# ohsnyt/bzip2-rust

Hardware: AMD Instinct MI355X
Metric: compress MB/s at -9 (900 KB blocks), 1/2/4/8 MI355X; bit-exact vs C bzip2 (higher is better)
Workload: dtype u8; 1 GPU; 1024 MiB per GPU synthetic text at -9 (1194 blocks on this rank), BASELINE configs[2]; raw_bytes_total=1073741824, blocks_rank0=1194, compressed_bytes=323302688

## Files before the change

### bzip2-rust_amd/csrc/bzx_api.hip

```cpp
#include <string.h>
#include <chrono>
#include <new>
#include "bzx_host.h"
#include "bzx_wg.h"

extern "C" const char *bzx_version(void) { return "bzx 0.1 (gfx950)"; }

extern "C" const char *bzx_strerror(int code)
{
    switch (code) {
    case BZX_OK: return "ok";
    case BZX_E_NODEVICE: return "no HIP device";
    case BZX_E_PARAM: return "bad parameter";
    case BZX_E_NOMEM: return "out of memory";
    case BZX_E_OUTBUF: return "output buffer too small";
    case BZX_E_HIP: return "HIP runtime error";
    case BZX_E_STATE: return "bad call sequence";
    case BZX_E_DATA: return "damaged or invalid bzip2 data";
    default: return "unknown error";
    }
}

extern "C" const char *bzx_last_error(const bzx_ctx *ctx) { return ctx ? ctx->err.c_str() : ""; }

// ... 31 lines not shown
    if (nslab <= ctx->cap_slabs) return BZX_OK;
    ctx->slabs.clear();
    ctx->cap_slabs = 0;
    const uint32_t cap = nslab < 16 ? 16 : nslab;
    if ((rc = dev_alloc(ctx, ctx->slabs, &ctx->d_in, (size_t)cap * BZX_BLK_STRIDE))) return rc;
    if ((rc = dev_alloc(ctx, ctx->slabs, &B.bwt, (size_t)cap * BZX_BLK_STRIDE))) return rc;
    if ((rc = dev_alloc(ctx, ctx->slabs, &B.rank, (size_t)cap * BZX_BLK_STRIDE))) return rc;
    if ((rc = dev_alloc(ctx, ctx->slabs, &B.mtfv, (size_t)cap * BZX_BLK_STRIDE))) return rc;
    if ((rc = dev_alloc(ctx, ctx->slabs, &B.freq, (size_t)cap * 260))) return rc;
    if ((rc = dev_alloc(ctx, ctx->slabs, &B.in_use, (size_t)cap * 256))) return rc;
    if ((rc = dev_alloc(ctx, ctx->slabs, &B.len, (size_t)cap * 6 * 260))) return rc;
    if ((rc = dev_alloc(ctx, ctx->slabs, &B.code, (size_t)cap * 6 * 260))) return rc;
    if ((rc = dev_alloc(ctx, ctx->slabs, &B.selector, (size_t)cap * BZX_SEL_STRIDE))) return rc;
    if ((rc = dev_alloc(ctx, ctx->slabs, &B.selector_mtf, (size_t)cap * BZX_SEL_STRIDE))) return rc;
    if ((rc = dev_alloc(ctx, ctx->slabs, &B.gbits, (size_t)cap * BZX_SEL_STRIDE))) return rc;
    if ((rc = dev_alloc(ctx, ctx->slabs, &B.pk, (size_t)cap * BZX_PK_STRIDE))) return rc;
    if ((rc = dev_alloc(ctx, ctx->slabs, &B.rec_a, (size_t)cap * BZX_MAX_N))) return rc;
    if ((rc = dev_alloc(ctx, ctx->slabs, &B.rec_b, (size_t)cap * BZX_MAX_N))) return rc;
    if ((rc = dev_alloc(ctx, ctx->slabs, &B.bk_list, (size_t)cap * BZX_BK_PER_BLOCK))) return rc;
    B.bk_cap = cap * BZX_BK_PER_BLOCK;
    if ((rc = dev_alloc(ctx, ctx->slabs, &B.rk_list, (size_t)B.bk_cap * 2))) return rc;
    if ((rc = dev_alloc(ctx, ctx->slabs, &B.deep_list, (size_t)cap * BZX_DEEP_PER_BLOCK * 4 * 3))) return rc;
    if ((rc = dev_alloc(ctx, ctx->slabs, &B.isa2, (size_t)cap * 2 * BZX_MAX_N))) return rc;
    B.rk_blocks = cap;
    B.hpos = reinterpret_cast<uint32_t *>(B.rec_a);
    B.hpos_stride = 2 * BZX_MAX_N;
    if ((rc = dev_alloc(ctx, ctx->slabs, &ctx->d_outbuf, (size_t)cap * (BZX_OUT_STRIDE / 4)))) return rc;
    ctx->cap_slabs = cap;
    return BZX_OK;
}
// ... 204 lines not shown
        Br.redo = 2;
        Br.ctr_bwt = BZX_CTR_RESUME_FETCH;
        bzx_launch_bwt(Br, grid_for(ctx, nblk, per_cu), ctx->stream);
        bzx_launch_periodic(B, ctx->n_slots < 64 ? ctx->n_slots : 64, ctx->stream);
    }
    HIP_TRY(ctx, hipEventRecord(ctx->ev[1], ctx->stream));
    if ((stages & STG_MTF) && nblk) bzx_launch_mtf(B, grid_for(ctx, nblk, 1), ctx->stream);
    HIP_TRY(ctx, hipEventRecord(ctx->ev[2], ctx->stream));
    if ((stages & STG_HUF) && nblk) bzx_launch_huffman(B, grid_for(ctx, nblk, 3), ctx->stream);
    HIP_TRY(ctx, hipEventRecord(ctx->ev[3], ctx->stream));
    if (stages & STG_EMIT) {
        if (out_level < 0) {
            B.out = (uint32_t *)d_stream_out;
            bzx_launch_layout(B, 0, 0, ctx->d_scalars, ctx->stream, d_phase);
            HIP_TRY(ctx, hipMemsetAsync(d_stream_out, 0, stream_cap, ctx->stream));
            if (nblk) bzx_launch_emit(B, grid_for(ctx, nblk, 2), ctx->stream);
        } else if (out_level == 0) {
            B.out = ctx->d_outbuf;
            bzx_launch_layout(B, 0, (uint64_t)BZX_OUT_STRIDE * 8, ctx->d_scalars, ctx->stream);
            HIP_TRY(ctx, hipMemsetAsync(ctx->d_outbuf, 0, (size_t)nblk * BZX_OUT_STRIDE, ctx->stream));
            if (nblk) bzx_launch_emit(B, grid_for(ctx, nblk, 2), ctx->stream);
        } else {
            B.out = (uint32_t *)d_stream_out;
            bzx_launch_layout(B, 32, 0, ctx->d_scalars, ctx->stream);
            HIP_TRY(ctx, hipMemcpyAsync(ctx->h_scalars, ctx->d_scalars, sizeof(uint64_t), hipMemcpyDeviceToHost,
                                        ctx->stream));
            HIP_TRY(ctx, hipStreamSynchronize(ctx->stream));
            const uint64_t out_bytes = (ctx->h_scalars[0] + 80 + 7) >> 3;
            const uint64_t need = (out_bytes + 3) & ~3ull;
            ctx->h_scalars[1] = out_bytes;
            if (need > stream_cap) {
                ctx->err = "output buffer too small for the compressed stream";
                return BZX_E_OUTBUF;
            }
            HIP_TRY(ctx, hipMemsetAsync(d_stream_out, 0, need, ctx->stream));
            if (nblk) bzx_launch_emit(B, grid_for(ctx, nblk, 2), ctx->stream);
            bzx_launch_stream_frame(B, out_level, ctx->d_scalars, ctx->d_scalars + 1, ctx->stream);
        }
    }
    HIP_TRY(ctx, hipEventRecord(ctx->ev[4], ctx->stream));
    HIP_TRY(ctx, hipMemcpyAsync(ctx->h_counters, ctx->d_counters, 64 * sizeof(uint32_t), hipMemcpyDeviceToHost, ctx->stream));
    HIP_TRY(ctx, hipGetLastError());
    return BZX_OK;
}

int bzx_ctx_split_scratch(bzx_ctx *ctx, size_t bytes, void **p)
{
    if (!ctx->split_ws.reserve(bytes)) {
        ctx->err = "hipMalloc(split scratch) failed";
        return BZX_E_NOMEM;
    }
// ... 639 lines not shown
    HIP_TRY(ctx, hipStreamSynchronize(ctx->stream));
    ctx->shard_packed_max = world <= 64 ? ctx->h_scalars[3] * 4 : 0;
    const uint64_t out_bytes = (ctx->h_scalars[0] + 80 + 7) >> 3;
    const uint64_t need = ctx->h_scalars[2] * 4;
    if (need > cap) {
        ctx->err = "packed buffer too small for this rank's blocks";
        return BZX_E_OUTBUF;
    }
    HIP_TRY(ctx, hipMemsetAsync(d_packed, 0, need, ctx->stream));
    HIP_TRY(ctx, hipMemsetAsync(ctx->d_counters, 0, 64 * sizeof(uint32_t), ctx->stream));
    B.out = (uint32_t *)d_packed;
    B.nblk = mine;
    B.blk_first = rank;
    B.blk_step = world;
    B.packed = 1;
    if (mine) bzx_launch_emit(B, grid_for(ctx, mine, 2), ctx->stream);
    B.packed = 0;
    HIP_TRY(ctx, hipEventRecord(ctx->ev[4], ctx->stream));
    HIP_TRY(ctx, hipEventRecord(ctx->ev[7], ctx->stream));
    if (nblk) HIP_TRY(ctx, hipMemcpyAsync(ctx->h_blk, B.blk, nblk * sizeof(BzxBlock), hipMemcpyDeviceToHost, ctx->stream));
    HIP_TRY(ctx, hipStreamSynchronize(ctx->stream));
    HIP_TRY(ctx, hipGetLastError());
    B.nblk = nblk;
    B.blk_first = 0;
    B.blk_step = 1;
    *packed_len = (size_t)need;
    *stream_len = (size_t)out_bytes;
    bzx_stats &st = ctx->stats;
    collect_stage_times(ctx);
    st.nblk = mine;
    ctx->stats_batch = false;
// ... 134 lines not shown
```

### bzip2-rust_amd/csrc/bzx_batch.hip

```cpp
#include <hip/hip_runtime.h>
#include <string.h>
#include <new>
#include "bzx_host.h"
#include "bzx_rle1.h"

#define BT_NT 1024
#define BX_NT 256
#define BX_WORDS 5
static_assert(sizeof(bzx_index_entry) == BX_WORDS * 8 && (BX_NT * BX_WORDS) % 2 == 0, "index entries: whole 16-byte vectors per workgroup");

__device__ __forceinline__ uint64_t bt_carry(const BzxBatchWs &ws, const BzxSeg &s, uint64_t tile)
{
    const uint64_t v = ws.tile_rs[tile], base = s.tile0 * RL_TILE;
    return v > base ? v - base : 0;
}

__global__ __launch_bounds__(RL_NT) void bzx_bt_runstart_kernel(BzxBatchWs ws)
{
    __shared__ uint64_t scratch[RL_NT / 64];
    for (uint64_t tile = blockIdx.x; tile < ws.ntiles; tile += gridDim.x) {
        const BzxSeg s = ws.seg[ws.tile_seg[tile]];
        bool any4;
        const uint64_t tot = bzx_tile_runstart(s.raw, s.len, tile - s.tile0, scratch, any4);
        if (threadIdx.x == 0) {
// ... 508 lines not shown
        }
        if (end > cap4) {
            ctx->err = "output buffer too small for the batch (input " + std::to_string(i0) + " onwards does not fit; "
                       "bzx_compress_batch_bound always fits)";
            return BZX_E_OUTBUF;
        }
        fold_blocks(stt, ctx->h_blk, 0, nb, 1);
        for (uint32_t i = i0; i < i1; i++) {
            stt.raw_bytes += lens[i];
            stt.out_bits += (uint64_t)out_lens[i] * 8;
        }
        stt.nblk += nb;
        HIP_TRY(ctx, hipEventRecord(ctx->ev_bt[1], st));
        HIP_TRY(ctx, hipMemsetAsync((uint8_t *)d_out + base, 0, end - base, st));
        B.nblk = nb;
        if (nb) bzx_launch_emit(B, grid_for(ctx, nb, 2), st);
        bzx_batch_launch_frame(ws, i0, i1, rb0, B.blk, d_out, level, st);
        HIP_TRY(ctx, hipEventRecord(ctx->ev_bt[2], st));
        HIP_TRY(ctx, hipGetLastError());
        emit_pending = true;
        base = end;
        i0 = i1;
    }
    HIP_TRY(ctx, hipEventRecord(ctx->ev[7], st));
    HIP_TRY(ctx, hipStreamSynchronize(st));
    if (emit_pending) {
        float ms = 0.f;
        (void)hipEventElapsedTime(&ms, ctx->ev_bt[1], ctx->ev_bt[2]);
        stt.ms_emit += ms;
    }
    (void)hipEventElapsedTime(&stt.ms_total, ctx->ev[5], ctx->ev[7]);
// ... 131 lines not shown
```

### bzip2-rust_amd/csrc/bzx_device.h

```cpp
#pragma once
#include <stdint.h>
#include <stddef.h>

#define BZX_MAX_N 900000u
#define BZX_BLK_STRIDE 900096u
#define BZX_MAX_ALPHA 258
#define BZX_G_SIZE 50
#define BZX_N_ITERS 4
#define BZX_MAX_SEL 18002
#define BZX_SEL_STRIDE 18048

#define BZX_IN_RAW (1ull << 63)
#define BZX_ST_PERIODIC 1u
#define BZX_ST_REDO 2u
#define BZX_ST_RESUME 4u
#define BZX_ST_DC_RANDOMISED 0x400u
#define DC_ERR_HEADER 0x100u
#define DC_ERR_DATA 0x200u
#define DC_SKIP 0x800u
#define DC_MAGIC_BLOCK 0x314159265359ull
#define DC_MAGIC_EOS 0x177245385090ull
#ifndef RK_ROUNDS
#define RK_ROUNDS 11
#endif
#define RK_COARSE 0x80000000u
// ... 71 lines not shown
    uint32_t *plist;
    const uint8_t *in;
    const uint8_t *raw;
    uint8_t *bwt;
    uint8_t *rank;
    uint32_t *hpos;
    uint32_t hpos_stride;
    uint16_t *mtfv;
    uint32_t *freq;
    uint8_t *in_use;
    uint8_t *len;
    uint32_t *code;
    uint8_t *selector;
    uint8_t *selector_mtf;
    uint16_t *gbits;
    uint32_t *out;
    BzxSortWs *sort_ws;
    uint8_t *pk;
    uint64_t *rec_a;
    uint64_t *rec_b;
    BzxBucket *bk_list;
    uint32_t bk_cap;
    uint32_t bk_affine;
    uint32_t *redo_list;
    uint32_t *resume_list;
    uint32_t *rk_list;
    uint32_t *deep_list;
    uint32_t deep_cap;
    uint32_t deep_lvl;
    uint32_t *isa2;
// ... 73 lines not shown
```

### bzip2-rust_amd/csrc/bzx_emit.hip

```cpp
#include <hip/hip_runtime.h>
#include "bzx_host.h"
#include "bzx_wg.h"

#define EMIT_NT 512
#define EMIT_NW (EMIT_NT / 64)

struct BitW {
    uint32_t *out;
    uint64_t wi;
    uint64_t acc;
    uint32_t nacc;
    bool first;
    __device__ __forceinline__ void init(uint32_t *o, uint64_t bitpos)
    {
        out = o;
        wi = bitpos >> 5;
        nacc = (uint32_t)(bitpos & 31u);
        acc = 0;
        first = true;
    }
    __device__ __forceinline__ void flush_word(uint32_t w)
    {
        const uint32_t be = __builtin_bswap32(w);
        if (first) {
            if (be) atomicOr(&out[wi], be);
            first = false;
        } else {
            out[wi] = be;
        }
        wi++;
    }
    __device__ __forceinline__ void put(uint32_t nbits, uint32_t val)
    {
        if (nbits == 0) return;
        acc = (acc << nbits) | (uint64_t)val;
        nacc += nbits;
        if (nacc >= 32) {
            nacc -= 32;
            flush_word((uint32_t)(acc >> nacc));
            acc &= (1ull << nacc) - 1ull;
        }
    }
    __device__ __forceinline__ void finish()
    {
        if (nacc > 0) {
            const uint32_t be = __builtin_bswap32((uint32_t)(acc << (32 - nacc)));
            if (be) atomicOr(&out[wi], be);
        }
    }
};

__shared__ uint8_t e_len[6][BZX_MAX_ALPHA + 2];
__shared__ uint32_t e_code[6][BZX_MAX_ALPHA + 2];
__shared__ uint32_t e_cl[6][BZX_MAX_ALPHA + 2];
__shared__ __attribute__((aligned(16))) uint32_t e_tile[EMIT_NT * (BZX_G_SIZE / 2)];
__shared__ uint32_t e_tabbits[8];
__shared__ uint32_t e_scratch[2 * EMIT_NW];
__shared__ uint32_t e_bcast[4];

#define EMIT_STAMP(slot)                                                      \
    do {                                                                      \
        if (B.dbg && tid == 0) {                                              \
            const unsigned long long now_ = wall_clock64();                   \
            atomicAdd(&B.dbg[slot], now_ - t_last);                           \
            t_last = now_;                                                    \
        }                                                                     \
    } while (0)

__global__ __launch_bounds__(EMIT_NT) void bzx_emit_kernel(BzxBatch B)
{
    const uint32_t tid = threadIdx.x, lane = bzx_lane(), wave = bzx_wave();
    unsigned long long t_last = 0;

    for (;;) {
        if (tid == 0) e_bcast[0] = atomicAdd(&B.counters[3], 1u);
        __syncthreads();
        const uint32_t j_ = e_bcast[0];
        __syncthreads();
        if (j_ >= B.nblk) break;
        const uint32_t b = B.blk_first + j_ * B.blk_step;

        if (B.dbg && tid == 0) t_last = wall_clock64();
        const BzxBlock d = B.blk[b];
        const uint32_t alpha = d.n_in_use + 2, n_mtf = d.n_mtf, n_sel = d.n_selectors, n_groups = d.n_groups;
        const uint16_t *__restrict__ V = B.mtfv + BZX_SLAB(B, b) * BZX_BLK_STRIDE;
        const uint8_t *__restrict__ SEL = B.selector + BZX_SLAB(B, b) * BZX_SEL_STRIDE;
        const uint8_t *__restrict__ SELM = B.selector_mtf + BZX_SLAB(B, b) * BZX_SEL_STRIDE;
        const uint16_t *__restrict__ GB = B.gbits + BZX_SLAB(B, b) * BZX_SEL_STRIDE;
        uint32_t *out = B.out;

        const uint64_t ob = B.packed ? d.pack_word * 32 + (d.out_bit & 31u) : d.out_bit;
        const uint64_t o_map = ob + 105;
        const uint64_t o_ng = o_map + d.sec_bits[3];
        const uint64_t o_sel = o_ng + 18;
        const uint64_t o_tab = o_sel + d.sec_bits[0];
        const uint64_t o_pay = o_tab + d.sec_bits[1];

        for (uint32_t i = tid; i < 6 * 260; i += EMIT_NT) {
            const uint32_t t = i / 260, v = i % 260;
            if (v < BZX_MAX_ALPHA + 2) {
                e_len[t][v] = B.len[BZX_SLAB(B, b) * 6 * 260 + i];
                e_code[t][v] = B.code[BZX_SLAB(B, b) * 6 * 260 + i];
                e_cl[t][v] = B.code[BZX_SLAB(B, b) * 6 * 260 + i] | ((uint32_t)B.len[BZX_SLAB(B, b) * 6 * 260 + i] << 24);
            }
        }
        __syncthreads();

        if (tid == 0) {
            BitW w;
            w.init(out, ob);
            w.put(24, 0x314159u);
            w.put(24, 0x265359u);
            w.put(32, d.crc);
            w.put(1, 0);
            w.put(24, d.orig_ptr);
            uint32_t l1 = 0, words[16];
            for (uint32_t i = 0; i < 16; i++) {
                uint32_t wv = 0;
                for (uint32_t j = 0; j < 16; j++)
                    if (B.in_use[BZX_SLAB(B, b) * 256 + i * 16 + j]) wv |= 0x8000u >> j;
                words[i] = wv;
                if (wv) l1 |= 0x8000u >> i;
            }
            w.put(16, l1);
            for (uint32_t i = 0; i < 16; i++)
                if (words[i]) w.put(16, words[i]);
            w.put(3, n_groups);
            w.put(15, n_sel);
            w.finish();
        }

        EMIT_STAMP(48);
        {
            const uint32_t per = (n_sel + EMIT_NT - 1) / EMIT_NT;
            const uint32_t lo = tid * per < n_sel ? tid * per : n_sel;
            const uint32_t hi = lo + per < n_sel ? lo + per : n_sel;
            uint32_t my_bits = 0;
            for (uint32_t i = lo; i < hi; i++) my_bits += SELM[i] + 1u;
            uint32_t tot;
            const uint32_t ex = bzx_block_excl_sum<EMIT_NT>(my_bits, e_scratch, tot);
            if (hi > lo) {
                BitW w;
                w.init(out, o_sel + ex);
                for (uint32_t i = lo; i < hi; i++) {
                    const uint32_t j = SELM[i];
                    w.put(j + 1, ((1u << j) - 1u) << 1);
                }
                w.finish();
            }
        }

        EMIT_STAMP(49);
        if (lane == 0 && wave < n_groups) {
            uint32_t bits = 5;
            int32_t curr = e_len[wave][0];
            for (uint32_t i = 0; i < alpha; i++) {
                const int32_t l = e_len[wave][i];
                bits += 2u * (uint32_t)(l > curr ? l - curr : curr - l) + 1u;
                curr = l;
            }
            e_tabbits[wave] = bits;
        }
        __syncthreads();
        if (lane == 0 && wave < n_groups) {
            uint64_t pos = o_tab;
            for (uint32_t t = 0; t < wave; t++) pos += e_tabbits[t];
            BitW w;
            w.init(out, pos);
            int32_t curr = e_len[wave][0];
            w.put(5, (uint32_t)curr);
            for (uint32_t i = 0; i < alpha; i++) {
                const int32_t l = e_len[wave][i];
                while (curr < l) {
                    w.put(2, 2);
                    curr++;
                }
                while (curr > l) {
                    w.put(2, 3);
                    curr--;
                }
                w.put(1, 0);
            }
            w.finish();
        }

        __syncthreads();
        EMIT_STAMP(50);
        {
            if (tid == 0) e_bcast[1] = 0;
            __syncthreads();
            for (uint32_t g0 = 0; g0 < n_sel; g0 += EMIT_NT) {
                const uint32_t g = g0 + tid;
                const uint32_t carry = e_bcast[1];
                const uint32_t gb = g < n_sel ? (uint32_t)GB[g] : 0u;
                uint32_t tot;
                const uint32_t ex = bzx_block_excl_sum<EMIT_NT>(gb, e_scratch, tot);
                {
                    const uint4 *__restrict__ src = reinterpret_cast<const uint4 *>(V + (size_t)g0 * BZX_G_SIZE);
                    uint4 *dst = reinterpret_cast<uint4 *>(e_tile);
                    const uint32_t ng = n_sel - g0 < EMIT_NT ? n_sel - g0 : EMIT_NT;
                    const uint32_t nq = (ng * (BZX_G_SIZE / 2) + 3u) / 4u;
                    for (uint32_t i = tid; i < nq; i += EMIT_NT) dst[i] = src[i];
                }
                __syncthreads();
                if (g < n_sel) {
                    const uint32_t gs = g * BZX_G_SIZE;
                    const uint32_t cnt = (n_mtf - gs < BZX_G_SIZE) ? n_mtf - gs : BZX_G_SIZE;
                    const uint32_t *vp = e_tile + tid * (BZX_G_SIZE / 2);
                    const uint32_t *__restrict__ cl = e_cl[SEL[g]];
                    uint32_t vw[BZX_G_SIZE / 2];
#pragma unroll
                    for (uint32_t k = 0; k < BZX_G_SIZE / 2; k++) vw[k] = 2 * k < cnt ? vp[k] : 0u;
                    BitW w;
                    w.init(out, o_pay + carry + ex);
#pragma unroll
                    for (uint32_t k = 0; k < BZX_G_SIZE / 2; k++) {
                        const uint32_t c0 = 2 * k < cnt ? cl[vw[k] & 0xffffu] : 0u;
                        const uint32_t c1 = 2 * k + 1 < cnt ? cl[vw[k] >> 16] : 0u;
                        w.put(c0 >> 24, c0 & 0xffffffu);
                        w.put(c1 >> 24, c1 & 0xffffffu);
                    }
                    w.finish();
                }
                if (tid == 0) e_bcast[1] = carry + tot;
                __syncthreads();
            }
        }
        __syncthreads();
        EMIT_STAMP(51);
    }
}

__global__ __launch_bounds__(EMIT_NT) void bzx_layout_kernel(BzxBatch B, uint64_t first_bit, uint64_t stride_bits,
                                                            uint64_t *total, uint64_t *phase)
{
    __shared__ uint64_t l_wsum[EMIT_NW];
    __shared__ uint64_t l_carry;
    const uint32_t tid = threadIdx.x, lane = bzx_lane(), wave = bzx_wave();
    if (phase) first_bit = phase[0];
    if (tid == 0) l_carry = first_bit;
    __syncthreads();
    for (uint32_t b0 = 0; b0 < B.nblk; b0 += EMIT_NT) {
        const uint32_t b = b0 + tid;
        const uint64_t v = b < B.nblk ? B.blk[b].bits : 0ull;
        uint64_t x = v;
// ... 169 lines not shown
void bzx_launch_unpack(const BzxBatch &B, const uint32_t *packed, uint32_t first, uint32_t step, uint32_t nown,
                       uint32_t grid, hipStream_t stream)
{
    hipLaunchKernelGGL(bzx_unpack_kernel, dim3(grid), dim3(256), 0, stream, B, packed, first, step, nown);
}

void bzx_launch_bits_export(const BzxBatch &B, long long *bits, hipStream_t stream)
{
    hipLaunchKernelGGL(bzx_bits_export_kernel, dim3(64), dim3(256), 0, stream, B, bits);
}
void bzx_launch_bits_import(const BzxBatch &B, const long long *bits, hipStream_t stream)
{
    hipLaunchKernelGGL(bzx_bits_import_kernel, dim3(64), dim3(256), 0, stream, B, bits);
}

void bzx_launch_emit(const BzxBatch &B, uint32_t grid, hipStream_t stream)
{
    hipLaunchKernelGGL(bzx_emit_kernel, dim3(grid), dim3(EMIT_NT), 0, stream, B);
}

void bzx_launch_layout(const BzxBatch &B, uint64_t first_bit, uint64_t stride_bits, uint64_t *d_total_bits,
                       hipStream_t stream, uint64_t *d_phase)
{
    hipLaunchKernelGGL(bzx_layout_kernel, dim3(1), dim3(EMIT_NT), 0, stream, B, first_bit, stride_bits, d_total_bits,
                       d_phase);
}

void bzx_launch_stream_frame(const BzxBatch &B, int level, const uint64_t *d_total_bits, uint64_t *d_out_bytes,
                             hipStream_t stream)
{
    hipLaunchKernelGGL(bzx_stream_frame_kernel, dim3(1), dim3(256), 0, stream, B, level, d_total_bits, d_out_bytes);
}
// ... 1 lines not shown
```

### bzip2-rust_amd/csrc/bzx_host.h

```cpp
#pragma once
#include <hip/hip_runtime.h>
#include <condition_variable>
#include <mutex>
#include <string>
#include <vector>
#include "../../include/bzx.h"
#include "bzx_dc.h"
#include "bzx_device.h"
#include "bzx_mem.h"

struct BlockReq {
    const uint8_t *blk;
    size_t n;
    uint32_t crc;
    uint8_t *out;
    size_t cap;
    size_t out_len = 0;
    uint8_t pad = 0;
    int rc = 0;
    bool done = false;
};

struct bzx_ctx {
    int device = 0;
// ... 163 lines not shown
__host__ __device__ static inline uint32_t crc_fold(uint32_t comb, uint32_t crc) { return ((comb << 1) | (comb >> 31)) ^ crc; }

void bzx_launch_shift_bits(const uint32_t *d_in, uint32_t n_words, uint32_t p, uint32_t *d_out, uint32_t n_cu,
                           hipStream_t stream);

void bzx_launch_bwt(const BzxBatch &B, uint32_t grid, hipStream_t stream);
uint32_t bzx_bwt_max_blocks_per_cu();
void bzx_launch_bsplit(const BzxBatch &B, uint32_t grid, uint32_t grid_deep, hipStream_t stream);
void bzx_launch_bsort(const BzxBatch &B, uint32_t grid, hipStream_t stream);
void bzx_launch_brank(const BzxBatch &B, uint32_t grid, hipStream_t stream);
void bzx_launch_bgiant(const BzxBatch &B, uint32_t grid, hipStream_t stream);
uint32_t bzx_bsort_blocks_per_cu();
void bzx_launch_periodic(const BzxBatch &B, uint32_t grid, hipStream_t stream);
void bzx_launch_mtf(const BzxBatch &B, uint32_t grid, hipStream_t stream);
void bzx_launch_huffman(const BzxBatch &B, uint32_t grid, hipStream_t stream);
void bzx_launch_emit(const BzxBatch &B, uint32_t grid, hipStream_t stream);
void bzx_launch_layout(const BzxBatch &B, uint64_t first_bit, uint64_t stride_bits, uint64_t *d_total_bits,
                       hipStream_t stream, uint64_t *d_phase = nullptr);
void bzx_launch_stream_frame(const BzxBatch &B, int level, const uint64_t *d_total_bits, uint64_t *d_out_bytes,
                             hipStream_t stream);
void bzx_launch_bits_export(const BzxBatch &B, long long *bits, hipStream_t stream);
void bzx_launch_bits_import(const BzxBatch &B, const long long *bits, hipStream_t stream);
void bzx_launch_pack_layout(const BzxBatch &B, uint32_t first, uint32_t step, uint32_t nown, uint64_t *d_total,
                            hipStream_t stream);
void bzx_launch_pack_max(const BzxBatch &B, uint32_t world, uint64_t *d_out, hipStream_t stream);
void bzx_launch_zero_edges(const BzxBatch &B, const uint64_t *d_total, hipStream_t stream);
void bzx_launch_unpack(const BzxBatch &B, const uint32_t *packed, uint32_t first, uint32_t step, uint32_t nown,
                       uint32_t grid, hipStream_t stream);

int bzx_split_launch_boundaries(bzx_ctx *ctx, const uint8_t *d_raw, size_t len, int level, uint32_t max_blocks,
                                BzxSplitWs *ws_out);
// ... 18 lines not shown
```

### bzip2-rust_amd/csrc/bzx_huff.hip

```cpp
#include <hip/hip_runtime.h>
#include "bzx_host.h"
#include "bzx_wg.h"

#define HUF_NT 512
#define HUF_NW (HUF_NT / 64)

__shared__ uint32_t h_freq[BZX_MAX_ALPHA + 2];
__shared__ uint8_t h_len[6][BZX_MAX_ALPHA + 2];
__shared__ uint2 h_lenAB[BZX_MAX_ALPHA + 2];
__shared__ uint32_t h_rfreq[6][BZX_MAX_ALPHA + 2];
#define HUF_PK 9
#define HUF_PK_COPIES 8
#define HUF_PK_STRIDE 19
__shared__ unsigned long long h_pk[HUF_PK_COPIES * HUF_PK_STRIDE];
__shared__ __attribute__((aligned(16))) uint64_t h_heap[6][BZX_MAX_ALPHA + 2];
__shared__ int32_t h_weight[6][BZX_MAX_ALPHA + 2];
__shared__ int32_t h_parent[6][BZX_MAX_ALPHA * 2];
__shared__ uint32_t h_code[6][BZX_MAX_ALPHA + 2];
__shared__ uint32_t h_part[6][2];
__shared__ uint32_t h_scratch[2 * HUF_NW];
__shared__ uint32_t h_bcast[4];
__shared__ uint32_t h_acc[4];

__device__ void make_code_lengths(int t, int32_t alpha, int32_t max_len)
{
    uint64_t *heap = h_heap[t];
    int32_t *weight = h_weight[t], *parent = h_parent[t];
    const int32_t lane = (int32_t)bzx_lane();
    for (int32_t i = lane; i < alpha; i += 64) {
        const uint32_t f = h_rfreq[t][i];
        weight[i + 1] = (int32_t)((f == 0 ? 1u : f) << 8);
    }
    for (;;) {
        bzx_wave_sync();
        if (lane == 0) {
            int32_t n_nodes = alpha, n_heap = 0;
            heap[0] = 0;
// ... 86 lines not shown
#ifdef BZX_HIP_EMU
#define HUF_FORGET(x) do {} while (0)
#else
#define HUF_FORGET(x) asm volatile("" : "+v"(x))
#endif

#define HUF_STAMP(slot)                                                       \
    do {                                                                      \
        if (B.dbg && tid == 0) {                                              \
            const unsigned long long now_ = wall_clock64();                   \
            atomicAdd(&B.dbg[slot], now_ - t_last);                           \
            t_last = now_;                                                    \
        }                                                                     \
    } while (0)

#ifndef HUF_WAVES_PER_SIMD
#define HUF_WAVES_PER_SIMD 6
#endif
__global__ __launch_bounds__(HUF_NT) __attribute__((amdgpu_waves_per_eu(HUF_WAVES_PER_SIMD, HUF_WAVES_PER_SIMD))) void bzx_huff_kernel(BzxBatch B)
{
    const uint32_t tid = threadIdx.x, lane = bzx_lane(), wave = bzx_wave();
    unsigned long long t_last = 0;

    for (;;) {
        if (tid == 0) h_bcast[0] = atomicAdd(&B.counters[2], 1u);
        __syncthreads();
        const uint32_t j_ = bzx_uni(h_bcast[0]);
        __syncthreads();
        if (j_ >= B.nblk) break;
        const uint32_t b = B.blk_first + j_ * B.blk_step;

        if (B.dbg && tid == 0) t_last = wall_clock64();
        const uint32_t n_mtf = bzx_uni(B.blk[b].n_mtf);
        const uint32_t alpha = bzx_uni(B.blk[b].n_in_use) + 2;
        const uint16_t *__restrict__ V = B.mtfv + BZX_SLAB(B, b) * BZX_BLK_STRIDE;
        uint8_t *__restrict__ SEL = B.selector + BZX_SLAB(B, b) * BZX_SEL_STRIDE;
        uint8_t *__restrict__ SELM = B.selector_mtf + BZX_SLAB(B, b) * BZX_SEL_STRIDE;
        uint16_t *__restrict__ GB = B.gbits + BZX_SLAB(B, b) * BZX_SEL_STRIDE;
        const uint32_t n_sel = (n_mtf + BZX_G_SIZE - 1) / BZX_G_SIZE;
        const uint32_t n_groups = n_mtf < 200 ? 2u : n_mtf < 600 ? 3u : n_mtf < 1200 ? 4u : n_mtf < 2400 ? 5u : 6u;

        for (uint32_t i = tid; i < BZX_MAX_ALPHA + 2; i += HUF_NT) h_freq[i] = i < alpha ? B.freq[BZX_SLAB(B, b) * 260 + i] : 0u;
        if (tid < 4) h_acc[tid] = 0;
        __syncthreads();

        if (tid == 0) {
            int32_t n_part = (int32_t)n_groups, rem_f = (int32_t)n_mtf, gs = 0;
            while (n_part > 0) {
                const int32_t t_freq = rem_f / n_part;
                int32_t ge = gs - 1, a_freq = 0;
                while (a_freq < t_freq && ge < (int32_t)alpha - 1) {
                    ge++;
                    a_freq += (int32_t)h_freq[ge];
// ... 139 lines not shown
                for (int k = 0; k < BZX_G_SIZE; k++) {
                    const uint32_t sm = (sy[k >> 1] >> (16 * (k & 1))) & 0xffffu;
                    const uint2 l2 = h_lenAB[sm];
                    accA += l2.x;
                    accB += l2.y;
                }
                const uint32_t pick = bt < 3 ? accA : accB;
                const uint32_t acc = (pick >> (10 * (bt % 3))) & 1023u;
                GB[g] = (uint16_t)acc;
                my_bits += acc;
            }
            uint32_t tot;
            (void)bzx_block_excl_sum<HUF_NT>(my_bits, h_scratch, tot);
            if (tid == 0) h_acc[2] = tot;
        }

        HUF_STAMP(44);
        {
            const uint32_t per = (n_sel + HUF_NT - 1) / HUF_NT;
            const uint32_t lo = tid * per;
            const uint32_t hi = lo + per < n_sel ? lo + per : n_sel;
            uint32_t lp[6] = {0, 0, 0, 0, 0, 0};
            for (uint32_t i = lo; i < hi; i++) {
                const uint32_t sg = SEL[i];
#pragma unroll
                for (uint32_t t = 0; t < 6; t++)
                    if (sg == t) lp[t] = i + 1;
            }
#pragma unroll
            for (uint32_t t = 0; t < 6; t++) {
// ... 71 lines not shown
```

### include/bzx.h

```cpp
#ifndef BZX_H
#define BZX_H

#include <stddef.h>
#include <stdint.h>

#ifdef __cplusplus
extern "C" {
#endif

#define BZX_OK 0
#define BZX_E_NODEVICE (-1)
#define BZX_E_PARAM (-2)
#define BZX_E_NOMEM (-3)
#define BZX_E_OUTBUF (-4)
#define BZX_E_HIP (-5)
#define BZX_E_STATE (-6)
#define BZX_E_DATA (-7)

#define BZX_MAX_BLOCK 900000u

typedef struct bzx_ctx bzx_ctx;

const char *bzx_version(void);
const char *bzx_strerror(int code);
// ... 8 lines not shown
int bzx_compress_blocks(bzx_ctx *ctx, uint32_t nblk, const uint8_t *const *blks, const size_t *ns,
                        const uint32_t *crcs, uint8_t *const *outs, const size_t *caps, size_t *out_lens,
                        uint8_t *pads);

int bzx_stage_bwt(bzx_ctx *ctx, const uint8_t *blk, size_t n, uint8_t *bwt_out, uint32_t *orig_ptr,
                  uint32_t *status);
int bzx_stage_mtf(bzx_ctx *ctx, const uint8_t *bwt, size_t n, uint16_t *mtfv_out, uint32_t *n_mtf,
                  uint32_t freq_out[258], uint8_t in_use_out[256]);
int bzx_stage_huffman(bzx_ctx *ctx, const uint16_t *mtfv, uint32_t n_mtf, const uint32_t freq[258],
                      uint32_t alpha_size, uint32_t *n_groups, uint32_t *n_selectors, uint8_t *selectors,
                      uint8_t len_out[6][258], uint32_t code_out[6][258]);
struct bzx_block_info;
int bzx_stage_encode(bzx_ctx *ctx, const uint16_t *mtfv, uint32_t n_mtf, const uint32_t freq[258],
                     const uint8_t in_use[256], uint32_t orig_ptr, uint32_t crc, uint8_t *out, size_t cap,
                     size_t *out_len, uint8_t *pad_bits, uint8_t *selector_mtf, struct bzx_block_info *info);

int bzx_split_rle1(bzx_ctx *ctx, const uint8_t *raw, size_t len, int level, uint8_t *blocks_out,
                   uint32_t nblk_cap, uint32_t *ns, uint32_t *crcs, uint32_t *nblk);

int bzx_compress_device(bzx_ctx *ctx, const void *d_raw, size_t len, int level, void *d_out, size_t cap,
                        size_t *out_len);
int bzx_compress_buffer(bzx_ctx *ctx, const uint8_t *raw, size_t len, int level, uint8_t *out, size_t cap,
                        size_t *out_len);

size_t bzx_compress_batch_bound(uint32_t count, const size_t *lens);
int bzx_compress_batch_device(bzx_ctx *ctx, uint32_t count, const void *const *d_raws, const size_t *lens, int level,
                              void *d_out, size_t cap, size_t *out_offs, size_t *out_lens);
int bzx_compress_batch_buffer(bzx_ctx *ctx, uint32_t count, const uint8_t *const *raws, const size_t *lens, int level,
                              uint8_t *out, size_t cap, size_t *out_offs, size_t *out_lens);

// ... 203 lines not shown
```

Before: 30240 MB/s.

## Split emit into per-tile work items with LDS-staged bit packing

The Huffman kernel now computes per-tile prefix bit offsets for each block. With those offsets, the emit kernel can split a block into several independent work items of four 512-group tiles each, instead of one workgroup serially walking all tiles. Each tile is packed into an LDS staging buffer without global atomics, then written out as byteswapped vector stores, with atomics only at the boundary words. The next tile's inputs are prefetched into registers, and the grid is capped at two workgroups per CU. In exchange, there is extra LDS use and the code tables are reloaded once per work item.

```diff
diff --git a/bzip2-rust_amd/csrc/bzx_api.hip b/bzip2-rust_amd/csrc/bzx_api.hip
--- a/bzip2-rust_amd/csrc/bzx_api.hip
+++ b/bzip2-rust_amd/csrc/bzx_api.hip
@@ -69,6 +69,7 @@
     if ((rc = dev_alloc(ctx, ctx->slabs, &B.selector, (size_t)cap * BZX_SEL_STRIDE))) return rc;
     if ((rc = dev_alloc(ctx, ctx->slabs, &B.selector_mtf, (size_t)cap * BZX_SEL_STRIDE))) return rc;
     if ((rc = dev_alloc(ctx, ctx->slabs, &B.gbits, (size_t)cap * BZX_SEL_STRIDE))) return rc;
+    if ((rc = dev_alloc(ctx, ctx->slabs, &B.tbits, (size_t)cap * BZX_TILE_STRIDE))) return rc;
     if ((rc = dev_alloc(ctx, ctx->slabs, &B.pk, (size_t)cap * BZX_PK_STRIDE))) return rc;
     if ((rc = dev_alloc(ctx, ctx->slabs, &B.rec_a, (size_t)cap * BZX_MAX_N))) return rc;
     if ((rc = dev_alloc(ctx, ctx->slabs, &B.rec_b, (size_t)cap * BZX_MAX_N))) return rc;
@@ -303,12 +304,12 @@
             B.out = (uint32_t *)d_stream_out;
             bzx_launch_layout(B, 0, 0, ctx->d_scalars, ctx->stream, d_phase);
             HIP_TRY(ctx, hipMemsetAsync(d_stream_out, 0, stream_cap, ctx->stream));
-            if (nblk) bzx_launch_emit(B, grid_for(ctx, nblk, 2), ctx->stream);
+            if (nblk) bzx_launch_emit(B, (uint32_t)ctx->n_cu, ctx->stream);
         } else if (out_level == 0) {
             B.out = ctx->d_outbuf;
             bzx_launch_layout(B, 0, (uint64_t)BZX_OUT_STRIDE * 8, ctx->d_scalars, ctx->stream);
             HIP_TRY(ctx, hipMemsetAsync(ctx->d_outbuf, 0, (size_t)nblk * BZX_OUT_STRIDE, ctx->stream));
-            if (nblk) bzx_launch_emit(B, grid_for(ctx, nblk, 2), ctx->stream);
+            if (nblk) bzx_launch_emit(B, (uint32_t)ctx->n_cu, ctx->stream);
         } else {
             B.out = (uint32_t *)d_stream_out;
             bzx_launch_layout(B, 32, 0, ctx->d_scalars, ctx->stream);
@@ -323,7 +324,7 @@
                 return BZX_E_OUTBUF;
             }
             HIP_TRY(ctx, hipMemsetAsync(d_stream_out, 0, need, ctx->stream));
-            if (nblk) bzx_launch_emit(B, grid_for(ctx, nblk, 2), ctx->stream);
+            if (nblk) bzx_launch_emit(B, (uint32_t)ctx->n_cu, ctx->stream);
             bzx_launch_stream_frame(B, out_level, ctx->d_scalars, ctx->d_scalars + 1, ctx->stream);
         }
     }
@@ -993,7 +994,7 @@
     B.blk_first = rank;
     B.blk_step = world;
     B.packed = 1;
-    if (mine) bzx_launch_emit(B, grid_for(ctx, mine, 2), ctx->stream);
+    if (mine) bzx_launch_emit(B, (uint32_t)ctx->n_cu, ctx->stream);
     B.packed = 0;
     HIP_TRY(ctx, hipEventRecord(ctx->ev[4], ctx->stream));
     HIP_TRY(ctx, hipEventRecord(ctx->ev[7], ctx->stream));
diff --git a/bzip2-rust_amd/csrc/bzx_batch.hip b/bzip2-rust_amd/csrc/bzx_batch.hip
--- a/bzip2-rust_amd/csrc/bzx_batch.hip
+++ b/bzip2-rust_amd/csrc/bzx_batch.hip
@@ -546,7 +546,7 @@
         HIP_TRY(ctx, hipEventRecord(ctx->ev_bt[1], st));
         HIP_TRY(ctx, hipMemsetAsync((uint8_t *)d_out + base, 0, end - base, st));
         B.nblk = nb;
-        if (nb) bzx_launch_emit(B, grid_for(ctx, nb, 2), st);
+        if (nb) bzx_launch_emit(B, (uint32_t)ctx->n_cu, st);
         bzx_batch_launch_frame(ws, i0, i1, rb0, B.blk, d_out, level, st);
         HIP_TRY(ctx, hipEventRecord(ctx->ev_bt[2], st));
         HIP_TRY(ctx, hipGetLastError());
diff --git a/bzip2-rust_amd/csrc/bzx_device.h b/bzip2-rust_amd/csrc/bzx_device.h
--- a/bzip2-rust_amd/csrc/bzx_device.h
+++ b/bzip2-rust_amd/csrc/bzx_device.h
@@ -9,6 +9,10 @@
 #define BZX_N_ITERS 4
 #define BZX_MAX_SEL 18002
 #define BZX_SEL_STRIDE 18048
+#define BZX_EMIT_TILE 512u
+#define BZX_MAX_TILES ((BZX_MAX_SEL + BZX_EMIT_TILE - 1) / BZX_EMIT_TILE)
+#define BZX_TILE_STRIDE 40
+static_assert(BZX_MAX_TILES <= BZX_TILE_STRIDE, "a block's tile prefixes fit its stride of BzxBatch.tbits");
 
 #define BZX_IN_RAW (1ull << 63)
 #define BZX_ST_PERIODIC 1u
@@ -110,6 +114,7 @@
     uint8_t *selector;
     uint8_t *selector_mtf;
     uint16_t *gbits;
+    uint32_t *tbits;
     uint32_t *out;
     BzxSortWs *sort_ws;
     uint8_t *pk;
diff --git a/bzip2-rust_amd/csrc/bzx_emit.hip b/bzip2-rust_amd/csrc/bzx_emit.hip
--- a/bzip2-rust_amd/csrc/bzx_emit.hip
+++ b/bzip2-rust_amd/csrc/bzx_emit.hip
@@ -5,7 +5,15 @@
 #define EMIT_NT 512
 #define EMIT_NW (EMIT_NT / 64)
 
-struct BitW {
+#ifndef EMIT_TPI
+#define EMIT_TPI 4
+#endif
+#define EMIT_SLOTS ((BZX_MAX_TILES + EMIT_TPI - 1) / EMIT_TPI)
+static_assert(EMIT_NT == BZX_EMIT_TILE, "one lane per group of a tile");
+#define EMIT_STAGE_BITS (EMIT_NT * BZX_G_SIZE * 17u)
+#define EMIT_STAGE_WORDS ((EMIT_STAGE_BITS / 32u + 2u + 3u + 3u) & ~3u)
+
+template <bool GLOBAL> struct BitWT {
     uint32_t *out;
     uint64_t wi;
     uint64_t acc;
@@ -21,7 +29,7 @@
     }
     __device__ __forceinline__ void flush_word(uint32_t w)
     {
-        const uint32_t be = __builtin_bswap32(w);
+        const uint32_t be = GLOBAL ? __builtin_bswap32(w) : w;
         if (first) {
             if (be) atomicOr(&out[wi], be);
             first = false;
@@ -44,16 +52,17 @@
     __device__ __forceinline__ void finish()
     {
         if (nacc > 0) {
-            const uint32_t be = __builtin_bswap32((uint32_t)(acc << (32 - nacc)));
+            const uint32_t w = (uint32_t)(acc << (32 - nacc));
+            const uint32_t be = GLOBAL ? __builtin_bswap32(w) : w;
             if (be) atomicOr(&out[wi], be);
         }
     }
 };
+typedef BitWT<true> BitW;
 
 __shared__ uint8_t e_len[6][BZX_MAX_ALPHA + 2];
-__shared__ uint32_t e_code[6][BZX_MAX_ALPHA + 2];
 __shared__ uint32_t e_cl[6][BZX_MAX_ALPHA + 2];
-__shared__ __attribute__((aligned(16))) uint32_t e_tile[EMIT_NT * (BZX_G_SIZE / 2)];
+__shared__ __attribute__((aligned(16))) uint32_t e_stage[EMIT_STAGE_WORDS];
 __shared__ uint32_t e_tabbits[8];
 __shared__ uint32_t e_scratch[2 * EMIT_NW];
 __shared__ uint32_t e_bcast[4];
@@ -67,18 +76,51 @@
         }                                                                     \
     } while (0)
 
+__device__ __forceinline__ void emit_load_tile(const uint16_t *__restrict__ V, const uint16_t *__restrict__ GB,
+                                               const uint8_t *__restrict__ SEL, const uint32_t *__restrict__ TB, uint32_t t,
+                                               uint32_t n_sel, uint32_t (&vw)[BZX_G_SIZE / 2], uint32_t &gb, uint32_t &sel,
+                                               uint32_t &tb)
+{
+    const uint32_t g = t * EMIT_NT + threadIdx.x;
+    tb = TB[t];
+    gb = 0;
+    sel = 0;
+#pragma unroll
+    for (uint32_t k = 0; k < BZX_G_SIZE / 2; k++) vw[k] = 0;
+    if (g < n_sel) {
+        const uint32_t *__restrict__ vp = reinterpret_cast<const uint32_t *>(V + (size_t)g * BZX_G_SIZE);
+#pragma unroll
+        for (uint32_t k = 0; k < BZX_G_SIZE / 2; k++) vw[k] = vp[k];
+        gb = GB[g];
+        sel = SEL[g];
+    }
+}
+
 __global__ __launch_bounds__(EMIT_NT) void bzx_emit_kernel(BzxBatch B)
 {
     const uint32_t tid = threadIdx.x, lane = bzx_lane(), wave = bzx_wave();
     unsigned long long t_last = 0;
+    const uint32_t n_items = B.nblk * EMIT_SLOTS;
+    uint4 *stage4 = reinterpret_cast<uint4 *>(e_stage);
+    for (uint32_t i = tid; i < EMIT_STAGE_WORDS / 4; i += EMIT_NT) stage4[i] = make_uint4(0u, 0u, 0u, 0u);
 
     for (;;) {
-        if (tid == 0) e_bcast[0] = atomicAdd(&B.counters[3], 1u);
-        __syncthreads();
-        const uint32_t j_ = e_bcast[0];
-        __syncthreads();
-        if (j_ >= B.nblk) break;
-        const uint32_t b = B.blk_first + j_ * B.blk_step;
+        if (tid == 0) {
+            uint32_t id;
+            for (;;) {
+                id = atomicAdd(&B.counters[3], 1u);
+                if (id >= n_items || id % EMIT_SLOTS == 0) break;
+                const uint32_t bb = B.blk_first + (id / EMIT_SLOTS) * B.blk_step;
+                if ((id % EMIT_SLOTS) * (EMIT_TPI * EMIT_NT) < B.blk[bb].n_selectors) break;
+            }
+            e_bcast[0] = id;
+        }
+        __syncthreads();
+        const uint32_t id = bzx_uni(e_bcast[0]);
+        __syncthreads();
+        if (id >= n_items) break;
+        const uint32_t slot = id % EMIT_SLOTS;
+        const uint32_t b = B.blk_first + (id / EMIT_SLOTS) * B.blk_step;
 
         if (B.dbg && tid == 0) t_last = wall_clock64();
         const BzxBlock d = B.blk[b];
@@ -87,6 +129,7 @@
         const uint8_t *__restrict__ SEL = B.selector + BZX_SLAB(B, b) * BZX_SEL_STRIDE;
         const uint8_t *__restrict__ SELM = B.selector_mtf + BZX_SLAB(B, b) * BZX_SEL_STRIDE;
         const uint16_t *__restrict__ GB = B.gbits + BZX_SLAB(B, b) * BZX_SEL_STRIDE;
+        const uint32_t *__restrict__ TB = B.tbits + BZX_SLAB(B, b) * BZX_TILE_STRIDE;
         uint32_t *out = B.out;
 
         const uint64_t ob = B.packed ? d.pack_word * 32 + (d.out_bit & 31u) : d.out_bit;
@@ -96,139 +139,164 @@
         const uint64_t o_tab = o_sel + d.sec_bits[0];
         const uint64_t o_pay = o_tab + d.sec_bits[1];
 
+        const uint32_t n_tiles = (n_sel + EMIT_NT - 1) / EMIT_NT;
+        const uint32_t t0 = slot * EMIT_TPI, t1 = t0 + EMIT_TPI < n_tiles ? t0 + EMIT_TPI : n_tiles;
         for (uint32_t i = tid; i < 6 * 260; i += EMIT_NT) {
             const uint32_t t = i / 260, v = i % 260;
             if (v < BZX_MAX_ALPHA + 2) {
-                e_len[t][v] = B.len[BZX_SLAB(B, b) * 6 * 260 + i];
-                e_code[t][v] = B.code[BZX_SLAB(B, b) * 6 * 260 + i];
-                e_cl[t][v] = B.code[BZX_SLAB(B, b) * 6 * 260 + i] | ((uint32_t)B.len[BZX_SLAB(B, b) * 6 * 260 + i] << 24);
-            }
-        }
-        __syncthreads();
-
-        if (tid == 0) {
-            BitW w;
-            w.init(out, ob);
-            w.put(24, 0x314159u);
-            w.put(24, 0x265359u);
-            w.put(32, d.crc);
-            w.put(1, 0);
-            w.put(24, d.orig_ptr);
-            uint32_t l1 = 0, words[16];
-            for (uint32_t i = 0; i < 16; i++) {
-                uint32_t wv = 0;
-                for (uint32_t j = 0; j < 16; j++)
-                    if (B.in_use[BZX_SLAB(B, b) * 256 + i * 16 + j]) wv |= 0x8000u >> j;
-                words[i] = wv;
-                if (wv) l1 |= 0x8000u >> i;
-            }
-            w.put(16, l1);
-            for (uint32_t i = 0; i < 16; i++)
-                if (words[i]) w.put(16, words[i]);
-            w.put(3, n_groups);
-            w.put(15, n_sel);
-            w.finish();
-        }
-
-        EMIT_STAMP(48);
-        {
-            const uint32_t per = (n_sel + EMIT_NT - 1) / EMIT_NT;
-            const uint32_t lo = tid * per < n_sel ? tid * per : n_sel;
-            const uint32_t hi = lo + per < n_sel ? lo + per : n_sel;
-            uint32_t my_bits = 0;
-            for (uint32_t i = lo; i < hi; i++) my_bits += SELM[i] + 1u;
-            uint32_t tot;
-            const uint32_t ex = bzx_block_excl_sum<EMIT_NT>(my_bits, e_scratch, tot);
-            if (hi > lo) {
+                const uint8_t l = B.len[BZX_SLAB(B, b) * 6 * 260 + i];
+                if (slot == 0) e_len[t][v] = l;
+                e_cl[t][v] = B.code[BZX_SLAB(B, b) * 6 * 260 + i] | ((uint32_t)l << 24);
+            }
+        }
+        uint32_t vn[BZX_G_SIZE / 2], gbn, seln, tbn;
+        emit_load_tile(V, GB, SEL, TB, t0, n_sel, vn, gbn, seln, tbn);
+        bzx_lds_barrier();
+
+        if (slot == 0) {
+            if (tid == 0) {
                 BitW w;
-                w.init(out, o_sel + ex);
-                for (uint32_t i = lo; i < hi; i++) {
-                    const uint32_t j = SELM[i];
-                    w.put(j + 1, ((1u << j) - 1u) << 1);
+                w.init(out, ob);
+                w.put(24, 0x314159u);
+                w.put(24, 0x265359u);
+                w.put(32, d.crc);
+                w.put(1, 0);
+                w.put(24, d.orig_ptr);
+                uint32_t l1 = 0, words[16];
+                for (uint32_t i = 0; i < 16; i++) {
+                    uint32_t wv = 0;
+                    for (uint32_t j = 0; j < 16; j++)
+                        if (B.in_use[BZX_SLAB(B, b) * 256 + i * 16 + j]) wv |= 0x8000u >> j;
+                    words[i] = wv;
+                    if (wv) l1 |= 0x8000u >> i;
                 }
+                w.put(16, l1);
+                for (uint32_t i = 0; i < 16; i++)
+                    if (words[i]) w.put(16, words[i]);
+                w.put(3, n_groups);
+                w.put(15, n_sel);
                 w.finish();
             }
-        }
-
-        EMIT_STAMP(49);
-        if (lane == 0 && wave < n_groups) {
-            uint32_t bits = 5;
-            int32_t curr = e_len[wave][0];
-            for (uint32_t i = 0; i < alpha; i++) {
-                const int32_t l = e_len[wave][i];
-                bits += 2u * (uint32_t)(l > curr ? l - curr : curr - l) + 1u;
-                curr = l;
-            }
-            e_tabbits[wave] = bits;
-        }
-        __syncthreads();
-        if (lane == 0 && wave < n_groups) {
-            uint64_t pos = o_tab;
-            for (uint32_t t = 0; t < wave; t++) pos += e_tabbits[t];
-            BitW w;
-            w.init(out, pos);
-            int32_t curr = e_len[wave][0];
-            w.put(5, (uint32_t)curr);
-            for (uint32_t i = 0; i < alpha; i++) {
-                const int32_t l = e_len[wave][i];
-                while (curr < l) {
-                    w.put(2, 2);
-                    curr++;
-                }
-                while (curr > l) {
-                    w.put(2, 3);
-                    curr--;
-                }
-                w.put(1, 0);
-            }
-            w.finish();
-        }
-
-        __syncthreads();
-        EMIT_STAMP(50);
-        {
-            if (tid == 0) e_bcast[1] = 0;
-            __syncthreads();
-            for (uint32_t g0 = 0; g0 < n_sel; g0 += EMIT_NT) {
-                const uint32_t g = g0 + tid;
-                const uint32_t carry = e_bcast[1];
-                const uint32_t gb = g < n_sel ? (uint32_t)GB[g] : 0u;
+
+            EMIT_STAMP(48);
+            {
+                const uint32_t per = (n_sel + EMIT_NT - 1) / EMIT_NT;
+                const uint32_t lo = tid * per < n_sel ? tid * per : n_sel;
+                const uint32_t hi = lo + per < n_sel ? lo + per : n_sel;
+                uint32_t my_bits = 0;
+                for (uint32_t i = lo; i < hi; i++) my_bits += SELM[i] + 1u;
                 uint32_t tot;
-                const uint32_t ex = bzx_block_excl_sum<EMIT_NT>(gb, e_scratch, tot);
-                {
-                    const uint4 *__restrict__ src = reinterpret_cast<const uint4 *>(V + (size_t)g0 * BZX_G_SIZE);
-                    uint4 *dst = reinterpret_cast<uint4 *>(e_tile);
-                    const uint32_t ng = n_sel - g0 < EMIT_NT ? n_sel - g0 : EMIT_NT;
-                    const uint32_t nq = (ng * (BZX_G_SIZE / 2) + 3u) / 4u;
-                    for (uint32_t i = tid; i < nq; i += EMIT_NT) dst[i] = src[i];
-                }
-                __syncthreads();
-                if (g < n_sel) {
-                    const uint32_t gs = g * BZX_G_SIZE;
-                    const uint32_t cnt = (n_mtf - gs < BZX_G_SIZE) ? n_mtf - gs : BZX_G_SIZE;
-                    const uint32_t *vp = e_tile + tid * (BZX_G_SIZE / 2);
-                    const uint32_t *__restrict__ cl = e_cl[SEL[g]];
-                    uint32_t vw[BZX_G_SIZE / 2];
-#pragma unroll
-                    for (uint32_t k = 0; k < BZX_G_SIZE / 2; k++) vw[k] = 2 * k < cnt ? vp[k] : 0u;
+                const uint32_t ex = bzx_block_excl_sum_lds<EMIT_NT>(my_bits, e_scratch, tot);
+                if (hi > lo) {
                     BitW w;
-                    w.init(out, o_pay + carry + ex);
-#pragma unroll
-                    for (uint32_t k = 0; k < BZX_G_SIZE / 2; k++) {
-                        const uint32_t c0 = 2 * k < cnt ? cl[vw[k] & 0xffffu] : 0u;
-                        const uint32_t c1 = 2 * k + 1 < cnt ? cl[vw[k] >> 16] : 0u;
-                        w.put(c0 >> 24, c0 & 0xffffffu);
-                        w.put(c1 >> 24, c1 & 0xffffffu);
+                    w.init(out, o_sel + ex);
+                    for (uint32_t i = lo; i < hi; i++) {
+                        const uint32_t j = SELM[i];
+                        w.put(j + 1, ((1u << j) - 1u) << 1);
                     }
                     w.finish();
                 }
-                if (tid == 0) e_bcast[1] = carry + tot;
-                __syncthreads();
-            }
-        }
-        __syncthreads();
+            }
+
+            EMIT_STAMP(49);
+            if (lane == 0 && wave < n_groups) {
+                uint32_t bits = 5;
+                int32_t curr = e_len[wave][0];
+                for (uint32_t i = 0; i < alpha; i++) {
+                    const int32_t l = e_len[wave][i];
+                    bits += 2u * (uint32_t)(l > curr ? l - curr : curr - l) + 1u;
+                    curr = l;
+                }
+                e_tabbits[wave] = bits;
+            }
+            bzx_lds_barrier();
+            if (lane == 0 && wave < n_groups) {
+                uint64_t pos = o_tab;
+                for (uint32_t t = 0; t < wave; t++) pos += e_tabbits[t];
+                BitW w;
+                w.init(out, pos);
+                int32_t curr = e_len[wave][0];
+                w.put(5, (uint32_t)curr);
+                for (uint32_t i = 0; i < alpha; i++) {
+                    const int32_t l = e_len[wave][i];
+                    while (curr < l) {
+                        w.put(2, 2);
+                        curr++;
+                    }
+                    while (curr > l) {
+                        w.put(2, 3);
+                        curr--;
+                    }
+                    w.put(1, 0);
+                }
+                w.finish();
+            }
+            EMIT_STAMP(50);
+        }
+
+        for (uint32_t t = t0; t < t1; t++) {
+            uint32_t vw[BZX_G_SIZE / 2];
+#pragma unroll
+            for (uint32_t k = 0; k < BZX_G_SIZE / 2; k++) vw[k] = vn[k];
+            const uint32_t gb = gbn, sel = seln;
+            const uint64_t start = o_pay + bzx_uni(tbn);
+            if (t + 1 < t1) emit_load_tile(V, GB, SEL, TB, t + 1, n_sel, vn, gbn, seln, tbn);
+
+            uint32_t tot;
+            const uint32_t ex = bzx_block_excl_sum_lds<EMIT_NT>(gb, e_scratch, tot);
+            const uint64_t wbase = start >> 5;
+            const uint32_t phase = (uint32_t)(start & 31u);
+            const uint32_t off = (uint32_t)((uintptr_t)(out + wbase) >> 2) & 3u;
+            const uint32_t g = t * EMIT_NT + tid;
+            if (g < n_sel) {
+                const uint32_t gs = g * BZX_G_SIZE;
+                const uint32_t cnt = (n_mtf - gs < BZX_G_SIZE) ? n_mtf - gs : BZX_G_SIZE;
+                const uint32_t *__restrict__ cl = e_cl[sel];
+                BitWT<false> w;
+                w.init(e_stage, off * 32u + phase + ex);
+#pragma unroll
+                for (uint32_t k = 0; k < BZX_G_SIZE / 2; k++) {
+                    const uint32_t c0 = 2 * k < cnt ? cl[vw[k] & 0xffffu] : 0u;
+                    const uint32_t c1 = 2 * k + 1 < cnt ? cl[vw[k] >> 16] : 0u;
+                    w.put(c0 >> 24, c0 & 0xffffffu);
+                    w.put(c1 >> 24, c1 & 0xffffffu);
+                }
+                w.finish();
+            }
+            bzx_lds_barrier();
+            const uint32_t end = off + ((phase + tot + 31u) >> 5);
+            uint32_t *gbase = out + wbase - off;
+            for (uint32_t i0 = 4 * tid; i0 < end; i0 += 4 * EMIT_NT) {
+                const uint4 v = stage4[i0 / 4];
+                stage4[i0 / 4] = make_uint4(0u, 0u, 0u, 0u);
+                const uint32_t x[4] = {__builtin_bswap32(v.x), __builtin_bswap32(v.y), __builtin_bswap32(v.z),
+                                       __builtin_bswap32(v.w)};
+                if (i0 > off && i0 + 4 < end) {
+                    *reinterpret_cast<uint4 *>(gbase + i0) = make_uint4(x[0], x[1], x[2], x[3]);
+                } else {
+#pragma unroll
+                    for (uint32_t c = 0; c < 4; c++) {
+                        const uint32_t i = i0 + c;
+                        if (i < off || i >= end) continue;
+                        if (i == off || i + 1 == end) {
+                            if (x[c]) atomicOr(gbase + i, x[c]);
+                        } else {
+                            gbase[i] = x[c];
+                        }
+                    }
+                }
+            }
+            bzx_lds_barrier();
+        }
         EMIT_STAMP(51);
     }
+}
+
+extern "C" void bzx_emit_geometry(uint32_t *tile_groups, uint32_t *tiles_per_item, uint32_t *staging_bits)
+{
+    if (tile_groups) *tile_groups = EMIT_NT;
+    if (tiles_per_item) *tiles_per_item = EMIT_TPI;
+    if (staging_bits) *staging_bits = (EMIT_STAGE_WORDS - 4u) * 32u;
 }
 
 __global__ __launch_bounds__(EMIT_NT) void bzx_layout_kernel(BzxBatch B, uint64_t first_bit, uint64_t stride_bits,
@@ -428,8 +496,10 @@
     hipLaunchKernelGGL(bzx_bits_import_kernel, dim3(64), dim3(256), 0, stream, B, bits);
 }
 
-void bzx_launch_emit(const BzxBatch &B, uint32_t grid, hipStream_t stream)
-{
+void bzx_launch_emit(const BzxBatch &B, uint32_t n_cu, hipStream_t stream)
+{
+    const uint64_t slots = (uint64_t)B.nblk * EMIT_SLOTS;
+    const uint32_t grid = slots < 2ull * n_cu ? (uint32_t)slots : 2u * n_cu;
     hipLaunchKernelGGL(bzx_emit_kernel, dim3(grid), dim3(EMIT_NT), 0, stream, B);
 }
 
diff --git a/bzip2-rust_amd/csrc/bzx_host.h b/bzip2-rust_amd/csrc/bzx_host.h
--- a/bzip2-rust_amd/csrc/bzx_host.h
+++ b/bzip2-rust_amd/csrc/bzx_host.h
@@ -201,7 +201,7 @@
 void bzx_launch_periodic(const BzxBatch &B, uint32_t grid, hipStream_t stream);
 void bzx_launch_mtf(const BzxBatch &B, uint32_t grid, hipStream_t stream);
 void bzx_launch_huffman(const BzxBatch &B, uint32_t grid, hipStream_t stream);
-void bzx_launch_emit(const BzxBatch &B, uint32_t grid, hipStream_t stream);
+void bzx_launch_emit(const BzxBatch &B, uint32_t n_cu, hipStream_t stream);
 void bzx_launch_layout(const BzxBatch &B, uint64_t first_bit, uint64_t stride_bits, uint64_t *d_total_bits,
                        hipStream_t stream, uint64_t *d_phase = nullptr);
 void bzx_launch_stream_frame(const BzxBatch &B, int level, const uint64_t *d_total_bits, uint64_t *d_out_bytes,
diff --git a/bzip2-rust_amd/csrc/bzx_huff.hip b/bzip2-rust_amd/csrc/bzx_huff.hip
--- a/bzip2-rust_amd/csrc/bzx_huff.hip
+++ b/bzip2-rust_amd/csrc/bzx_huff.hip
@@ -21,6 +21,8 @@
 __shared__ uint32_t h_scratch[2 * HUF_NW];
 __shared__ uint32_t h_bcast[4];
 __shared__ uint32_t h_acc[4];
+__shared__ uint32_t h_tbits[BZX_MAX_TILES];
+static_assert(BZX_EMIT_TILE % 64 == 0 && BZX_MAX_TILES <= 64, "a wave sums whole 64-group pieces of a tile; one wave scans the tiles");
 
 __device__ void make_code_lengths(int t, int32_t alpha, int32_t max_len)
 {
@@ -137,6 +139,24 @@
         }                                                                     \
     } while (0)
 
+__device__ __attribute__((noinline)) void huff_tile_prefixes(const uint16_t *GB, uint32_t *TB, uint32_t n_sel)
+{
+    const uint32_t lane = bzx_lane(), wave = bzx_wave();
+    for (uint32_t tl = wave; tl < BZX_MAX_TILES; tl += HUF_NW) {
+        const uint32_t ge = (tl + 1) * BZX_EMIT_TILE < n_sel ? (tl + 1) * BZX_EMIT_TILE : n_sel;
+        uint32_t s = 0;
+        for (uint32_t g = tl * BZX_EMIT_TILE + lane; g < ge; g += 64) s += GB[g];
+        s = bzx_wave_incl_sum(s);
+        if (lane == 63) h_tbits[tl] = s;
+    }
+    __syncthreads();
+    if (wave == 0) {
+        const uint32_t tb = lane < BZX_MAX_TILES ? h_tbits[lane] : 0u;
+        const uint32_t incl = bzx_wave_incl_sum(tb);
+        if (lane < BZX_MAX_TILES) TB[lane] = incl - tb;
+    }
+}
+
 #ifndef HUF_WAVES_PER_SIMD
 #define HUF_WAVES_PER_SIMD 6
 #endif
@@ -160,6 +180,7 @@
         uint8_t *__restrict__ SEL = B.selector + BZX_SLAB(B, b) * BZX_SEL_STRIDE;
         uint8_t *__restrict__ SELM = B.selector_mtf + BZX_SLAB(B, b) * BZX_SEL_STRIDE;
         uint16_t *__restrict__ GB = B.gbits + BZX_SLAB(B, b) * BZX_SEL_STRIDE;
+        uint32_t *__restrict__ TB = B.tbits + BZX_SLAB(B, b) * BZX_TILE_STRIDE;
         const uint32_t n_sel = (n_mtf + BZX_G_SIZE - 1) / BZX_G_SIZE;
         const uint32_t n_groups = n_mtf < 200 ? 2u : n_mtf < 600 ? 3u : n_mtf < 1200 ? 4u : n_mtf < 2400 ? 5u : 6u;
 
@@ -329,6 +350,7 @@
             (void)bzx_block_excl_sum<HUF_NT>(my_bits, h_scratch, tot);
             if (tid == 0) h_acc[2] = tot;
         }
+        huff_tile_prefixes(GB, TB, n_sel);
 
         HUF_STAMP(44);
         {
diff --git a/include/bzx.h b/include/bzx.h
--- a/include/bzx.h
+++ b/include/bzx.h
@@ -46,6 +46,7 @@
 int bzx_stage_encode(bzx_ctx *ctx, const uint16_t *mtfv, uint32_t n_mtf, const uint32_t freq[258],
                      const uint8_t in_use[256], uint32_t orig_ptr, uint32_t crc, uint8_t *out, size_t cap,
                      size_t *out_len, uint8_t *pad_bits, uint8_t *selector_mtf, struct bzx_block_info *info);
+void bzx_emit_geometry(uint32_t *tile_groups, uint32_t *tiles_per_item, uint32_t *staging_bits);
 
 int bzx_split_rle1(bzx_ctx *ctx, const uint8_t *raw, size_t len, int level, uint8_t *blocks_out,
                    uint32_t nblk_cap, uint32_t *ns, uint32_t *crcs, uint32_t *nblk);
```

Result: faster. 31280 MB/s (median of 6 runs) (+3.4%).
